# uricchio/2DSFS-scan

Measured on AMD Instinct MI355X. Metric: genomic windows/s (T2D+T1D+Fst) at 20 kb, n1=n2=50; HBM GB/s fraction, higher is better.
Workload: dtype f64

## Files before the change

2dsfs-scan_amd/csrc/sfs2d_kernels.hpp:

```cpp
#pragma once

#include <type_traits>
#include <hip/hip_runtime.h>

#include <cmath>
#include <cstdint>

#include "sfs2d.h"

namespace sfs2dk {

constexpr int WAVE = 64;
constexpr int BLOCK = 256;
constexpr int SBLOCK = 512;
constexpr int BLOCK1 = 512;
constexpr int FBLOCK = 1024;
constexpr int KBLOCK = 512;
constexpr int LNX_N = 1 << 20;
constexpr int LNT = 512;
constexpr int LNF = 256;
__host__ __device__ inline int wl_rtn(int n1p, int n2p) { return 2 * (n1p > n2p ? n1p : n2p) + 2; }
constexpr int RCPN = 512;
#ifndef SFS2D_ABL
#define SFS2D_ABL 0
// ... 500 lines not shown
                                          uint2* __restrict__ slots, uint32_t* __restrict__ bins,
                                          uint32_t* __restrict__ bcount, uint32_t* __restrict__ err_word, int hr,
                                          const double2* __restrict__ rcp_g, unsigned long long* __restrict__ fsum) {
  __shared__ uint32_t sh_b2;
  __shared__ unsigned long long sh_fst[FST ? 2 * FST_R * FST_LDS : 1];
  __shared__ double2 sh_rcp[FST ? RCPN / 2 : 1];
  __shared__ uint32_t sh_wlo;
  static_assert(!JNT || (DO_BG && LDS_HIST && !DO_BINS && !FILT && !FST), "JNT: histogram / segmentation passes only");
  if (JNT) hr = 1;
  STAMP(20);
  BLK_STAMP(0, 0);
  uint32_t* gh = repl + ((size_t)(ti % REPL) * P.nchrom + t.chrom) * (size_t)P.nh;
  const int lane0 = threadIdx.x & (WAVE - 1);
  const int hsh = LDS_HIST ? (hr == 4 ? 2 : 0) : 0;
  const int rep = lane0 & (hr - 1);
  const int trash = P.nh * hr + lane0;
  if (FST) {
    for (int k = threadIdx.x; k < 2 * FST_R * FST_LDS; k += BLOCK1) sh_fst[k] = 0ull;
    for (int k = threadIdx.x; k < RCPN / 2; k += BLOCK1) sh_rcp[k] = rcp_g[k];
    if (threadIdx.x == 0) sh_wlo = DO_SEG ? wid_fast(P, pos[t.begin]) : div_fast(P, t.begin - t.cb);
  }
  if (DO_BG) {
    if (LDS_HIST) {
      const int nz = P.nh * hr + WAVE + (JNT ? P.nb2 : 0);
      uint4* const z4 = reinterpret_cast<uint4*>(sh_hist);
      for (int k = threadIdx.x; k < (nz >> 2); k += BLOCK1) z4[k] = make_uint4(0u, 0u, 0u, 0u);
      if ((int)threadIdx.x < (nz & 3)) sh_hist[(nz & ~3) + (int)threadIdx.x] = 0u;
    }
    if (threadIdx.x == 0) sh_b2 = 0u;
  }
  if (DO_SEG) {
    const uint32_t wf = wid_fast(P, pos[t.begin]);
    const uint32_t lo = t.begin == t.cb ? 0u : wf + 1u;
    const uint32_t hi = t.end == t.ce ? t.nslots : wid_fast(P, pos[t.end]);
    for (uint32_t s = lo + threadIdx.x; s < hi; s += BLOCK1)
      if (s != wf) slots[(size_t)t.sbase + s] = make_uint2(0u, 0u);
  }
  if (DO_BG || FST || DO_SEG) __syncthreads();
  const uint32_t wlo = FST ? sh_wlo : 0u;
  const int frep = threadIdx.x & (FST_R - 1);
  auto fst_add = [&](uint32_t wid, double num, double den) {
    const unsigned long long qn = fst_fixed(num, P.fst_scale), qd = fst_fixed(den, P.fst_scale);
    if ((qn | qd) == 0ull) return;
    const uint32_t j = wid - wlo;
    if (j < (uint32_t)FST_LDS) {
      atomicAdd(&sh_fst[2 * (j * FST_R + frep)], qn);
      atomicAdd(&sh_fst[2 * (j * FST_R + frep) + 1], qd);
    } else {
      atomicAdd(&fsum[2 * ((size_t)t.sbase + wid)], qn);
      atomicAdd(&fsum[2 * ((size_t)t.sbase + wid) + 1], qd);
    }
  };
  const bool pos_filter = FILT && (P.has_start || P.has_end);
  const bool need_pos = DO_SEG || pos_filter;
  const bool filt = FILT && P.ann_want >= 0;
  const int lane = threadIdx.x & (WAVE - 1);
  uint32_t err = 0, b2 = 0;
  STAMP(21);

  KParams Q = P;
  if (!JNT) {
    Q.n1 = vreg(P.n1); Q.n2 = vreg(P.n2); Q.n1p = vreg(P.n1p); Q.n2p = vreg(P.n2p); Q.nb2 = vreg(P.nb2);
    Q.fold_thr = vreg(P.fold_thr); Q.h1a = vreg(P.h1a); Q.h1b = vreg(P.h1b);
    Q.wmag = vreg(P.wmag); Q.wsh1 = vreg(P.wsh1); Q.wsh2 = vreg(P.wsh2);
  }
  auto process = [&](auto EDGE_C, auto FAST_C, uint32_t i0, const uint4& cv, const uint4& pv, const uint2& av,
                     uint32_t wprev, uint32_t wnext) {
    constexpr bool EDGE = decltype(EDGE_C)::value, FAST = decltype(FAST_C)::value;
    const uint32_t cc[4] = {cv.x, cv.y, cv.z, cv.w};
    const uint32_t pp[4] = {pv.x, pv.y, pv.z, pv.w};
    const uint32_t aa[4] = {av.x & 0xffffu, av.x >> 16, av.y & 0xffffu, av.y >> 16};
    uint32_t w[4];
    if (DO_SEG) {
#pragma unroll
      for (int k = 0; k < 4; ++k) w[k] = wid_fast(Q, pp[k]);
    }
    uint32_t bw[4];
    uint32_t segcode = 0;
    uint32_t fw[4];
    bool fm[4];
#pragma unroll
    for (int k = 0; k < 4; ++k) {
      const uint32_t i = i0 + k;
      const bool in = EDGE ? (i >= t.begin) & (i < t.end) : true;
      bool var_ok = in, pos_ok = true;
      if (filt) var_ok = in & ((int)aa[k] == P.ann_want);
      if (pos_filter) {
        const long long p = (long long)pp[k];
        pos_ok = (!P.has_start | (p >= P.start_pos)) & (!P.has_end | (p <= P.end_pos));
      }
      int k2all, u1a, u1b;
      bw[k] = FAST ? classify_fast(Q, cc[k], var_ok, pos_ok, k2all, u1a, u1b)
                   : classify(P, cc[k], var_ok, pos_ok, err, k2all, u1a, u1b);
      if (FST) {
        fw[k] = DO_SEG ? w[k] : div_fast(Q, i - t.cb);
        fm[k] = in & (k2all >= 0) & (DO_SEG | (fw[k] < t.nslots));
      }
      if (DO_BG) {
        if (LDS_HIST) {
          atomicAdd(&sh_hist[(in & (k2all >= 0)) ? (k2all << hsh) + rep : trash], 1u);
          atomicAdd(&sh_hist[(in & (u1a >= 0)) ? ((Q.h1a + u1a) << hsh) + rep : trash], 1u);
          atomicAdd(&sh_hist[(in & (u1b >= 0)) ? ((Q.h1b + u1b) << hsh) + rep : trash], 1u);
        } else if (in) {
          if (k2all >= 0) atomicAdd(&gh[k2all], 1u);
          if (u1a >= 0) atomicAdd(&gh[P.h1a + u1a], 1u);
          if (u1b >= 0) atomicAdd(&gh[P.h1b + u1b], 1u);
        }
        b2 += (in & (bin_k2(bw[k]) != 0)) ? 1u : 0u;
      }
      if (DO_SEG) {
        const uint32_t qp = k ? w[k - 1] : wprev;
        const uint32_t qn = k < 3 ? w[k + 1] : wnext;
        const bool first = in & ((i == t.cb) | (qp != w[k]));
        const bool last = in & ((i + 1 == t.ce) | (qn != w[k]));
        segcode |= (first ? 1u : 0u) << (2 * k) | (last ? 2u : 0u) << (2 * k);
      }
      __builtin_amdgcn_sched_barrier(0);
    }
    if (FST) {
#pragma unroll
      for (int k = 0; k < 4; ++k) {
        double nk, dk;
        fst_snp(cc[k], fm[k], rcp_g, nk, dk);
        if (fm[k]) fst_add(fw[k], nk, dk);
      }
    }
    if (DO_SEG && segcode) {
      for (uint32_t c = segcode; c; c &= c - 1) {
        const int bit = __builtin_ctz(c), k = bit >> 1;
        const uint32_t wk = k == 0 ? w[0] : k == 1 ? w[1] : k == 2 ? w[2] : w[3];
        uint32_t* sl = reinterpret_cast<uint32_t*>(slots + ((size_t)t.sbase + wk));
        sl[bit & 1] = i0 + k + 1u;
      }
    }
    if (DO_BINS) {
      if (!EDGE || (i0 >= t.begin && i0 + 4 <= t.end)) {
        *reinterpret_cast<uint4*>(bins + i0) = make_uint4(bw[0], bw[1], bw[2], bw[3]);
      } else {
#pragma unroll
        for (int k = 0; k < 4; ++k)
          if (i0 + k >= t.begin && i0 + k < t.end) bins[i0 + k] = bw[k];
      }
    }
  };

  constexpr bool FASTOK = !FILT && (!DO_BG || LDS_HIST);
  const uint32_t s2 = (uint32_t)hsh + 2u;
  uint32_t* const hist_l = sh_hist + rep;
  uint32_t* const h1a_l = hist_l + ((uint32_t)P.h1a << hsh);
  uint32_t* const h1b_l = hist_l + ((uint32_t)P.h1b << hsh);
  uint32_t* const trash_p = sh_hist + trash;
  uint32_t* const jh_l = sh_hist + P.nh * hr + WAVE;
  const uint32_t n2p1 = vreg(P.n2 + 1), nb2m1 = vreg(P.nb2 - 1), n1pm1 = vreg(P.n1p - 1), n2pm1 = vreg(P.n2p - 1);
  auto process_fast = [&](uint32_t i0, const uint4& cv, const uint4& pv, uint32_t wprev, uint32_t wnext) {
    const uint32_t cc[4] = {cv.x, cv.y, cv.z, cv.w};
    const uint32_t pp[4] = {pv.x, pv.y, pv.z, pv.w};
    uint32_t w[4], bw[4];
    if (DO_SEG) {
#pragma unroll
      for (int k = 0; k < 4; ++k) w[k] = wid_fast(Q, pp[k]);
    }
    uint32_t fw[4];
    bool fm[4];
#pragma unroll
    for (int k = 0; k < 4; ++k) {
      uint32_t c = cc[k];
      asm volatile("" : "+v"(c));
      const uint32_t r1 = c & 0xffu, a1 = (c >> 8) & 0xffu, r2 = (c >> 16) & 0xffu, a2 = c >> 24;
      const bool sw = (int)(a1 + a2) > Q.fold_thr;
      const uint32_t x1 = sw ? r1 : a1, x2 = sw ? r2 : a2;
      const uint32_t k2 = __umul24(x1, n2p1) + x2;
      const bool in2 = k2 != 0u, last = k2 == nb2m1;
      const uint32_t g1 = min(a1, (uint32_t)Q.n1 - a1), g2 = min(a2, (uint32_t)Q.n2 - a2);
      const uint32_t f1 = g1 - 1u < n1pm1 ? g1 : 0u, f2 = g2 - 1u < n2pm1 ? g2 : 0u;
      bw[k] = (last ? B_LAST : k2) | (f1 << 16) | (f2 << 23) | B_VAR;
      if (DO_BG && !(SFS2D_ABL & 64)) {
        atomicAdd(in2 ? (uint32_t*)((char*)hist_l + (k2 << s2)) : trash_p, 1u);
        atomicAdd(a1 ? (uint32_t*)((char*)h1a_l + (a1 << s2)) : trash_p, 1u);
        atomicAdd(a2 ? (uint32_t*)((char*)h1b_l + (a2 << s2)) : trash_p, 1u);
        b2 += (in2 & !last) ? 1u : 0u;
      }
      if (FST) {
        fw[k] = DO_SEG ? w[k] : div_fast(Q, i0 + k - t.cb);
        fm[k] = in2 & (DO_SEG | (fw[k] < t.nslots));
      }
    }
    if (FST) {
      double sn = 0.0, sd = 0.0;
      uint32_t wc = fw[0];
#pragma unroll
      for (int k = 0; k < 4; ++k) {
        double nk, dk;
        fst_snp(cc[k], fm[k], sh_rcp, nk, dk);
        if (k && fw[k] != wc) {
          fst_add(wc, sn, sd);
          sn = 0.0; sd = 0.0; wc = fw[k];
        }
        sn += nk; sd += dk;
      }
      fst_add(wc, sn, sd);
    }
    if (DO_SEG && wprev != wnext) {
#pragma unroll
      for (int k = 0; k < 4; ++k) {
        const uint32_t qp = k ? w[k - 1] : wprev, qn = k < 3 ? w[k + 1] : wnext;
        uint32_t* sl = reinterpret_cast<uint32_t*>(slots + ((size_t)t.sbase + w[k]));
        if (qp != w[k]) sl[0] = i0 + k + 1u;
        if (qn != w[k]) sl[1] = i0 + k + 1u;
      }
    }
    if (DO_BINS) *reinterpret_cast<uint4*>(bins + i0) = make_uint4(bw[0], bw[1], bw[2], bw[3]);
  };

  constexpr uint32_t LSNP = 4;
  typedef __attribute__((address_space(3))) uint32_t lds_u32;
  const uint32_t kmA = vreg(P.kmul << 8), kmR = P.kmul, fthr = (uint32_t)P.fold_thr;
  const uint32_t jhb = vreg((uint32_t)(uintptr_t)((lds_u32*)jh_l)), h2b = vreg((uint32_t)(uintptr_t)((lds_u32*)sh_hist));
  auto jnt_fast = [&](uint32_t i0, const uint4& cv, const uint4& pv, uint32_t wprev, uint32_t wnext) {
    const uint32_t cc[4] = {cv.x, cv.y, cv.z, cv.w};
    const uint32_t pp[4] = {pv.x, pv.y, pv.z, pv.w};
    if (!(SFS2D_ABL & 64)) {
      uint32_t ka[4], kr[4], sm[4];
#pragma unroll
      for (int k = 0; k < 4; ++k) {
        ka[k] = __builtin_amdgcn_udot4(cc[k], kmA, 0u, false);
        kr[k] = __builtin_amdgcn_udot4(cc[k], kmR, 0u, false);
        sm[k] = __builtin_amdgcn_udot4(cc[k], 0x01000100u, 0u, false);
      }
      asm volatile("" : "+v"(ka[0]), "+v"(ka[1]), "+v"(ka[2]), "+v"(ka[3]), "+v"(kr[0]), "+v"(kr[1]), "+v"(kr[2]),
                        "+v"(kr[3]), "+v"(sm[0]), "+v"(sm[1]), "+v"(sm[2]), "+v"(sm[3]));
#pragma unroll
      for (int k = 0; k < 4; ++k) {
        if (ka[k] != 0u)
          __hip_atomic_fetch_add((lds_u32*)(uintptr_t)(jhb + (ka[k] << 2)), 1u, __ATOMIC_RELAXED, __HIP_MEMORY_SCOPE_WORKGROUP);
        if (((int)sm[k] > (int)fthr) & (kr[k] != 0u))
          __hip_atomic_fetch_add((lds_u32*)(uintptr_t)(h2b + (kr[k] << 2)), 1u, __ATOMIC_RELAXED, __HIP_MEMORY_SCOPE_WORKGROUP);
      }
    }
    if (DO_SEG && wprev != wnext) {
      uint32_t w[LSNP];
#pragma unroll
      for (int k = 0; k < (int)LSNP; ++k) w[k] = wid_fast(P, pp[k]);
#pragma unroll
      for (int k = 0; k < (int)LSNP; ++k) {
        const uint32_t qp = k ? w[k - 1] : wprev, qn = k < (int)LSNP - 1 ? w[k + 1] : wnext;
        uint32_t* sl = reinterpret_cast<uint32_t*>(slots + ((size_t)t.sbase + w[k]));
        if (qp != w[k]) sl[0] = i0 + k + 1u;
        if (qn != w[k]) sl[1] = i0 + k + 1u;
      }
    }
  };

  constexpr uint32_t STEP = LSNP * BLOCK1;
  const uint32_t ab = t.begin & ~3u, alast = (t.end - 1u) & ~3u;
  constexpr bool NEED_C = DO_BG || DO_BINS || FST;
  struct StepIn {
    uint4 c, p;
    uint2 a;
    uint32_t x;
  };
  const uint32_t tbytes = (alast + 4u - ab) * 4u;
  const __amdgpu_buffer_rsrc_t crs = __builtin_amdgcn_make_buffer_rsrc(const_cast<uint32_t*>(counts + ab), (short)0, (int)tbytes, 0x00020000);
  const __amdgpu_buffer_rsrc_t prs = __builtin_amdgcn_make_buffer_rsrc(const_cast<uint32_t*>(pos + ab), (short)0, (int)tbytes, 0x00020000);
  const __amdgpu_buffer_rsrc_t chr_rs =
      __builtin_amdgcn_make_buffer_rsrc(const_cast<uint32_t*>(pos + t.cb), (short)0, (int)((t.ce - t.cb) * 4u), 0x00020000);
  const int lane_off = (int)(LSNP * 4u * threadIdx.x);
  const uint32_t wave_snp = LSNP * WAVE * (uint32_t)__builtin_amdgcn_readfirstlane((int)(threadIdx.x >> 6));
  const uint32_t xlane_off = lane < WAVE / 2 ? 0u - 4u : LSNP * WAVE * 4u;
  auto load_step = [&](uint32_t base) {
    StepIn x;
    const int off = (int)(base - ab) * 4 + lane_off;
    x.c = NEED_C ? __builtin_bit_cast(uint4, __builtin_amdgcn_raw_buffer_load_b128(crs, off, 0, 0)) : make_uint4(0, 0, 0, 0);
    x.p = need_pos ? __builtin_bit_cast(uint4, __builtin_amdgcn_raw_buffer_load_b128(prs, off, 0, 0)) : make_uint4(0, 0, 0, 0);
    x.a = filt ? *reinterpret_cast<const uint2*>(ann + min(base + LSNP * threadIdx.x, alast)) : make_uint2(0, 0);
    x.x = 0;
    if (DO_SEG) {
      const uint32_t wb4 = base < t.end ? (base + wave_snp - t.cb) * 4u : (t.ce - t.cb) * 4u + 4u;
      x.x = __builtin_amdgcn_raw_buffer_load_b32(chr_rs, (int)(wb4 + xlane_off), 0, 0);
    }
    return x;
  };
  auto body = [&](uint32_t base, const StepIn& cur) {
    const uint32_t ia = base + LSNP * threadIdx.x;
    const uint2 aav = cur.a;
    const bool edge = base < t.begin || base + STEP > t.end || base <= t.cb || base + STEP >= t.ce;
    uint32_t wpa = 0, wna = 0;
    if (DO_SEG) {
      uint32_t pprev = dpp_keep<0x138>(cur.x, cur.p.w);
      uint32_t pnext = dpp_keep<0x130>(cur.x, cur.p.x);
      if (edge) {
        const uint32_t none = (t.ce - t.cb) * 4u;
        const uint32_t ni = ia + LSNP;
        const bool edge_next = lane == WAVE - 1 || ni >= t.end;
        const uint32_t op = (lane == 0 && ia > t.cb) ? (min(ia, alast + 4u) - 1u - t.cb) * 4u : none;
        const uint32_t on = (edge_next && ni < t.ce) ? (ni - t.cb) * 4u : none;
        const uint32_t xp = __builtin_amdgcn_raw_buffer_load_b32(chr_rs, (int)op, 0, 0);
        const uint32_t xn = __builtin_amdgcn_raw_buffer_load_b32(chr_rs, (int)on, 0, 0);
        if (lane == 0) pprev = xp;
        if (edge_next) pnext = xn;
      }
      wpa = wid_fast(P, pprev);
      wna = wid_fast(P, pnext);
    }
    auto nc1 = [](uint32_t c) { return __builtin_amdgcn_udot4(c, 0x00000101u, 0u, false); };
    auto nc2 = [](uint32_t c) { return __builtin_amdgcn_udot4(c, 0x01010000u, 0u, false); };
    auto any_bad = [&]() -> bool {
      const uint4 ca = cur.c;
      const uint32_t m1 = max(max(nc1(ca.x), nc1(ca.y)), max(nc1(ca.z), nc1(ca.w)));
      const uint32_t m2 = max(max(nc2(ca.x), nc2(ca.y)), max(nc2(ca.z), nc2(ca.w)));
      return __ballot((m1 > (uint32_t)P.n1) | (m2 > (uint32_t)P.n2)) != 0ull;
    };
    using T_ = std::true_type;
    using F_ = std::false_type;
    bool exact = !FASTOK || edge;
    int nc_ok = P.nc_ok;
    asm volatile("" : "+s"(nc_ok));
    if (!exact && !nc_ok) exact = any_bad();
    if (exact) process(T_{}, F_{}, ia, cur.c, cur.p, aav, wpa, wna);
    else {
#ifdef SFS2D_MARK
      asm volatile("; HOT_BEGIN");
#endif
      if (SFS2D_ABL & 128)
        asm volatile("" ::"v"(cur.c.x), "v"(cur.c.y), "v"(cur.c.z), "v"(cur.c.w), "v"(cur.p.x), "v"(cur.p.w), "v"(wpa), "v"(wna));
      else if constexpr (JNT) jnt_fast(ia, cur.c, cur.p, wpa, wna);
      else process_fast(ia, cur.c, cur.p, wpa, wna);
#ifdef SFS2D_MARK
      asm volatile("; HOT_END");
#endif
    }
  };
#if SFS2D_PREP_PREFETCH >= 2
  StepIn bufA = load_step(ab), bufB = load_step(ab + STEP);
  for (uint32_t base = ab; base < t.end; base += 2 * STEP) {
    body(base, bufA);
    bufA = load_step(base + 2 * STEP);
    if (base + STEP >= t.end) break;
    body(base + STEP, bufB);
    bufB = load_step(base + 3 * STEP);
  }
#else
  StepIn nxt = load_step(ab);
  for (uint32_t base = ab; base < t.end; base += STEP) {
#if SFS2D_PREP_PREFETCH
    const StepIn cur = nxt;
    if (base + STEP < t.end) nxt = load_step(base + STEP);
#else
    const StepIn cur = base == ab ? nxt : load_step(base);
#endif
    body(base, cur);
  }
#endif
  STAMP(22);
  if (err) atomicOr(err_word, err);
  if (DO_BG && !JNT) {
    b2 = wave_sum_u(b2);
    if (lane == 0 && b2) atomicAdd(&sh_b2, b2);
  }
  if (DO_BG || FST) __syncthreads();
  if (JNT) {
    const uint32_t n2p1 = (uint32_t)P.n2 + 1u;
    uint32_t bs = 0;
    for (int k = threadIdx.x; k < P.nb2; k += BLOCK1) {
      const uint32_t j = jh_l[k];
      const uint32_t x1 = __umulhi((uint32_t)k, P.n2inv), x2 = (uint32_t)k - x1 * n2p1;
      if (j) {
        if (x1) atomicAdd(&sh_hist[P.h1a + (int)x1], j);
        if (x2) atomicAdd(&sh_hist[P.h1b + (int)x2], j);
      }
      const uint32_t v = sh_hist[k] + ((int)(x1 + x2) <= P.fold_thr ? j : 0u);
      if (k) sh_hist[k] = v;
      if (k >= 1 && k <= P.nb2 - 2) bs += v;
    }
    bs = wave_sum_u(bs);
    if (lane == 0 && bs) atomicAdd(&sh_b2, bs);
    __syncthreads();
  }
  if (FST)
    for (int j = threadIdx.x; j < FST_LDS; j += BLOCK1) {
      unsigned long long qn = 0, qd = 0;
#pragma unroll
      for (int r = 0; r < FST_R; ++r) {
        qn += sh_fst[2 * (j * FST_R + r)];
        qd += sh_fst[2 * (j * FST_R + r) + 1];
      }
      if (qn | qd) {
        atomicAdd(&fsum[2 * ((size_t)t.sbase + wlo + j)], qn);
        atomicAdd(&fsum[2 * ((size_t)t.sbase + wlo + j) + 1], qd);
      }
    }
  if (DO_BG) {
    if (LDS_HIST)
      for (int k = threadIdx.x; k < P.nh; k += BLOCK1) {
        uint32_t v;
        if (hr == 4) {
// ... 1089 lines not shown
  __builtin_amdgcn_s_barrier();
#endif
  BLK_STAMP(1, 1);
}

template <int CTRL>
__device__ __forceinline__ double mdpp_d(double v) {
  const unsigned long long u = __double_as_longlong(v);
  const int lo = __builtin_amdgcn_mov_dpp((int)(u & 0xffffffffull), CTRL, 0xf, 0xf, false);
  const int hi = __builtin_amdgcn_mov_dpp((int)(u >> 32), CTRL, 0xf, 0xf, false);
  return __longlong_as_double((long long)(((unsigned long long)(uint32_t)hi << 32) | (uint32_t)lo));
}
__device__ __forceinline__ void wave_sum2_halves(double a, double b, double& s2, double& sa, double& sb) {
  a += mdpp_d<0xB1>(a);  b += mdpp_d<0xB1>(b);
  a += mdpp_d<0x4E>(a);  b += mdpp_d<0x4E>(b);
  a += mdpp_d<0x141>(a); b += mdpp_d<0x141>(b);
  a += mdpp_d<0x140>(a); b += mdpp_d<0x140>(b);
  s2 = (readlane_d(a, 0) + readlane_d(a, 16)) + (readlane_d(a, 32) + readlane_d(a, 48));
  sa = readlane_d(b, 0) + readlane_d(b, 16);
  sb = readlane_d(b, 32) + readlane_d(b, 48);
}
__device__ __forceinline__ double wave_sum1(double v) {
  v += mdpp_d<0xB1>(v);
  v += mdpp_d<0x4E>(v);
  v += mdpp_d<0x141>(v);
  v += mdpp_d<0x140>(v);
  return (readlane_d(v, 0) + readlane_d(v, 16)) + (readlane_d(v, 32) + readlane_d(v, 48));
}

__device__ __forceinline__ double swap16_d(double v, bool upper) {
  const unsigned long long u = __double_as_longlong(v);
  const auto lo = __builtin_amdgcn_permlane16_swap((uint32_t)(u & 0xffffffffull), (uint32_t)(u & 0xffffffffull), false, false);
  const auto hi = __builtin_amdgcn_permlane16_swap((uint32_t)(u >> 32), (uint32_t)(u >> 32), false, false);
  const uint32_t l = upper ? lo[1] : lo[0], h = upper ? hi[1] : hi[0];
  return __longlong_as_double((long long)(((unsigned long long)h << 32) | l));
}
__device__ __forceinline__ double swap32_d(double v, bool upper) {
  const unsigned long long u = __double_as_longlong(v);
  const auto lo = __builtin_amdgcn_permlane32_swap((uint32_t)(u & 0xffffffffull), (uint32_t)(u & 0xffffffffull), false, false);
  const auto hi = __builtin_amdgcn_permlane32_swap((uint32_t)(u >> 32), (uint32_t)(u >> 32), false, false);
  const uint32_t l = upper ? lo[1] : lo[0], h = upper ? hi[1] : hi[0];
  return __longlong_as_double((long long)(((unsigned long long)h << 32) | l));
}
__device__ __forceinline__ double row_sum_d(double v) {
  v += mdpp_d<0xB1>(v);
  v += mdpp_d<0x4E>(v);
  v += mdpp_d<0x141>(v);
  v += mdpp_d<0x140>(v);
  return v;
}
__device__ __forceinline__ double wave_sum_all(double v) {
  v = row_sum_d(v);
  v = swap16_d(v, false) + swap16_d(v, true);
  return swap32_d(v, false) + swap32_d(v, true);
}
__device__ __forceinline__ void wave_sum_halves_all(double v, double& a, double& b) {
  v = row_sum_d(v);
  v = swap16_d(v, false) + swap16_d(v, true);
  a = swap32_d(v, false);
  b = swap32_d(v, true);
}

__device__ __forceinline__ void swap32_pair(double x, double y, double& xo, double& yo) {
  const unsigned long long u = __double_as_longlong(x), v = __double_as_longlong(y);
  const auto lo = __builtin_amdgcn_permlane32_swap((uint32_t)u, (uint32_t)v, false, false);
  const auto hi = __builtin_amdgcn_permlane32_swap((uint32_t)(u >> 32), (uint32_t)(v >> 32), false, false);
  xo = __longlong_as_double((long long)(((unsigned long long)hi[0] << 32) | lo[0]));
  yo = __longlong_as_double((long long)(((unsigned long long)hi[1] << 32) | lo[1]));
}
__device__ __forceinline__ void swap16_pair(double x, double y, double& xo, double& yo) {
  const unsigned long long u = __double_as_longlong(x), v = __double_as_longlong(y);
  const auto lo = __builtin_amdgcn_permlane16_swap((uint32_t)u, (uint32_t)v, false, false);
  const auto hi = __builtin_amdgcn_permlane16_swap((uint32_t)(u >> 32), (uint32_t)(v >> 32), false, false);
  xo = __longlong_as_double((long long)(((unsigned long long)hi[0] << 32) | lo[0]));
  yo = __longlong_as_double((long long)(((unsigned long long)hi[1] << 32) | lo[1]));
}
__device__ __forceinline__ double wave_sum5(double a, double h, double f1, double f2, uint32_t lane) {
  double x, y;
  swap32_pair(a, f2, x, y);
  const double r1 = x + y;
  swap32_pair(f1, h, x, y);
  const double r2 = lane < 32 ? x + y : y;
  const double r3 = x;
  swap16_pair(r1, r2, x, y);
  const double q = x + y;
  swap16_pair(r3, r3, x, y);
  const double t = x + y;
  const bool odd = lane & 1u;
  double z = odd ? t : q;
  z += mdpp_d<0xB1>(odd ? q : t);
  z += mdpp_d<0x4E>(z);
  z += mdpp_d<0x124>(z);
  z += mdpp_d<0x128>(z);
  return z;
}

__device__ __forceinline__ void wave_sum3(double a, double b, double c, double& sa, double& sb, double& sc) {
  double x, y;
  swap32_pair(a, b, x, y);
  const double r1 = x + y;
  swap32_pair(c, c, x, y);
  const double r2 = x + y;
  swap16_pair(r1, r2, x, y);
  double q = x + y;
  q += mdpp_d<0xB1>(q);
  q += mdpp_d<0x4E>(q);
  q += mdpp_d<0x124>(q);
  q += mdpp_d<0x128>(q);
  sa = readlane_d(q, 0);
  sc = readlane_d(q, 16);
  sb = readlane_d(q, 32);
}

extern "C" __device__ int sfs2d_llvm_writelane(int v, int l, int old) __asm("llvm.amdgcn.writelane.i32");
__device__ __forceinline__ uint32_t wlane(uint32_t v, int l, uint32_t old) {
  return (uint32_t)sfs2d_llvm_writelane((int)__builtin_amdgcn_readfirstlane((int)v), l, (int)old);
}


__device__ __forceinline__ void lds_copy_d(double* dst, const double* __restrict__ src, int n) {
  constexpr int U = 8;
  for (int k0 = threadIdx.x; k0 < n; k0 += U * SBLOCK) {
    double v[U];
#pragma unroll
    for (int j = 0; j < U; ++j) v[j] = k0 + j * SBLOCK < n ? src[k0 + j * SBLOCK] : 0.0;
#pragma unroll
    for (int j = 0; j < U; ++j)
      if (k0 + j * SBLOCK < n) dst[k0 + j * SBLOCK] = v[j];
  }
}

template <bool P16, bool FUSED, int FST, bool CNT, bool GATE = false>
__device__ __forceinline__ void scan_w_small(double* ldsd, uint32_t wgi, uint32_t nwg, SCAN_W_ARGS) {
  constexpr bool FSTIN = FST >= 2;
  constexpr bool FMASK = FST == 3;
  static_assert(!FSTIN || CNT, "Fst in the scan reads the counts");
  static_assert(!GATE || CNT, "the gate is a property of the counts the scan classifies");
  constexpr int DT = LNT;
  constexpr int R1U = R1;
  constexpr int NWV = SBLOCK / WAVE;
  constexpr int SB = 8;
  __shared__ BgHead sh_hb;
  __shared__ double sh_bd[NWV][3][SB];
  __shared__ uint32_t sh_bu[NWV][5][SB];
  __shared__ unsigned long long sh_bf[NWV][FST ? 2 : 1][SB];
  STAMP(10);
  BLK_STAMP(1, 0);
  const int tid = threadIdx.x;
  const int wv = __builtin_amdgcn_readfirstlane(tid >> 6);
  const int lane = tid & (WAVE - 1);
  const Chunk ch = chunks[wgi];
  const int bg = bg_per_chrom ? (int)ch.chrom : 0;

  double* LPl = ldsd;
  double* Dt = LPl + ((P.nt + 1) & ~1);
  double* Ft = Dt + DT;
  double2* RT = reinterpret_cast<double2*>(Ft + LNF);
  const int rtn = FSTIN ? P.rtn : 0;
  uint32_t* HB = reinterpret_cast<uint32_t*>(RT + rtn);
  const int h2w = P16 ? ((P.nb2 + 1) / 2 + 3) & ~3 : (P.nb2 + 3) & ~3;
  const int h1w = R1 * (P.n1p + 1), h1wb = R1 * (P.n2p + 1);
  const int per = (h2w + h1w + h1wb + 3) & ~3;
  uint32_t* W = HB + wv * per;
  uint32_t* H1a = W + h2w;
  uint32_t* H1b = H1a + h1w;
  const uint32_t rep = lane & (R1U - 1);

  auto bounds = [&](uint32_t s, uint2 sr, Win& w, bool live) {
    if (mode_bp) {
      w.has = live && sr.x != 0u;
      w.b = sr.x - 1u;
      w.e = sr.y;
    } else {
      w.has = live;
      w.b = ch.cb + (ch.wid_lo + (s - ch.slot_lo)) * P.ws;
      w.e = w.b + P.ws;
    }
    const __amdgpu_buffer_rsrc_t rr = window_rows(bins, w.has ? w.b : 0u, w.has ? w.e : 0u, P.nm1);
    uint32_t lo = (uint32_t)lane * 4u;
    asm volatile("" : "+v"(lo));
#pragma unroll
    for (int j = 0; j < 8; ++j) w.u[j] = __builtin_amdgcn_raw_buffer_load_b32(rr, (int)lo + 256 * j, 0, 0);
  };
  uint32_t s = ch.slot_lo + ch.first + wv;
  const bool active = s < ch.slot_hi;
  const uint2 sr0 = (active && mode_bp) ? slots[s] : make_uint2(0, 0);
  const uint32_t npool = ch.pool & 0xffffu, pool = ch.pool >> 16;
  const bool dyn = ch.slot_lo + ch.nstatic < ch.slot_hi;
  const uint32_t dbase = ch.slot_lo + ch.nstatic + pool;
  uint32_t* myctr = ctr + (((size_t)cpar * P.nchrom + ch.chrom) * CTR_POOLS + pool) * CTR_STRIDE;
  uint32_t gq1 = 0, gq = 0;
  if (active && dyn && lane == 0) {
    gq1 = atomicAdd(myctr, 1u);
    gq = atomicAdd(myctr, 1u);
  }
  if (wgi == 0)
    for (int k = tid; k < P.nchrom * CTR_POOLS; k += SBLOCK) ctr[((size_t)(1 - cpar) * P.nchrom * CTR_POOLS + k) * CTR_STRIDE] = 0u;

  static_assert(LNT == SBLOCK && LNF <= SBLOCK, "one D and at most one F double per thread");
  const double dfv0 = dfg[tid], dfv1 = tid < LNF ? dfg[LNT + tid] : 0.0;
  const double2 rtv = (FSTIN && tid < rtn) ? reinterpret_cast<const double2*>(dfg + 2 * LNT)[tid] : make_double2(0.0, 0.0);
  auto stage_fst = [&]() {
    if (FSTIN && tid < rtn) RT[tid] = rtv;
  };
  BgHead hb;
  const size_t rs = (size_t)P.nchrom * P.nh;
  const uint32_t* Rc = repl + (size_t)par * REPL * rs + (size_t)ch.chrom * P.nh;
  if (!FUSED) {
    double lsv = 0.0;
    int4 my_node = make_int4(0, 0, -1, 0);
    uint32_t bc = 0u;
    Bg1D o{};
    if (sliced) {
      if (tid < nleaves) lsv = leafsum[(size_t)bg * nleaves + tid];
      if (tid < nnodes) my_node = nodes[tid];
      if (tid == 0) { bc = bcount[(size_t)par * P.nchrom + bg]; o = bg1d[bg]; }
    }
    lds_copy_d(LPl, LPg + (size_t)bg * P.nt, P.nt);
    if (tid < DT) Dt[tid] = dfv0;
    if (tid < LNF) Ft[tid] = dfv1;
    stage_fst();
    if (sliced) {
      const bool writer = ch.first == 0 && (int)ch.chrom == write_chrom;
      double* lsum = reinterpret_cast<double*>(HB);
      if (tid < nleaves) lsum[tid] = lsv;
      __syncthreads();
      for (int l = 0; l < nlevels; ++l) {
        if (my_node.z == l) lsum[nleaves + tid] = lsum[my_node.x] + lsum[my_node.y];
        __syncthreads();
      }
      if (tid == 0) {
        const double B2 = (double)bc;
        uint32_t flags = o.flags;
        if (B2 == 0.0) flags |= BGF_B2_ZERO;
        const int M2 = P.nb2 - 2;
        if (M2 >= 1 && B2 != 0.0) {
          const double S = (nleaves + nnodes) ? lsum[nleaves + nnodes - 1] : 0.0;
          const double padj = 1.0 - S;
          if (padj < -1e-15) {
            flags |= BGF_NAN2;
          } else if (fabs(padj) > 1e-15) {
            const double l2 = log(padj);
            LPl[M2] = l2;
            if (writer) { tab[(size_t)bg * P.nt + M2].lp = l2; LPg[(size_t)bg * P.nt + M2] = l2; }
          }
        }
        BgHead h;
        h.B2 = B2; h.B1a = o.B1a; h.B1b = o.B1b; h.flags = flags; h.pad = 0;
        sh_hb = h;
        if (writer) head[bg] = h;
      }
      if (wgi == 0)
        for (int c = tid; c < P.nchrom; c += SBLOCK) bcount[(size_t)(1 - par) * P.nchrom + c] = 0u;
      __syncthreads();
      hb = sh_hb;
    } else {
      hb = head[bg];
    }
  } else {
    if (tid < DT) Dt[tid] = dfv0;
    if (tid < LNF) Ft[tid] = dfv1;
    stage_fst();
    fused_table(P.nb2, P.nh, P.nt, P.n1p, P.n2p, P.n1, P.n2, P.t1a, P.t1b, P.nchrom, ch.chrom,
                ch.first == 0 && (int)ch.chrom == write_chrom, bg,
                Rc, rs, repl, bcount, par, tab, LPg, head, LPl, HB, leaves, nleaves, nodes, nnodes, nlevels, lnx,
                &sh_hb, reinterpret_cast<double*>(HB) + 1536, HB + FUSED_VCNT);
    hb = sh_hb;
  }
  for (int k = lane; k < per / 4; k += WAVE) reinterpret_cast<uint4*>(W)[k] = make_uint4(0, 0, 0, 0);
  if (tid == 0) LPl[0] = 0.0;
  __syncthreads();
  if (FUSED) {
    uint32_t* Ro = repl + (size_t)(1 - par) * REPL * rs;
    const size_t tot = (size_t)REPL * rs, share = (tot + nwg - 1) / nwg;
    const size_t lo = (size_t)wgi * share, hi = lo + share < tot ? lo + share : tot;
    for (size_t k = lo + tid; k < hi; k += SBLOCK) Ro[k] = 0u;
    if (wgi == 0)
      for (int c = tid; c < P.nchrom; c += SBLOCK) bcount[(size_t)(1 - par) * P.nchrom + c] = 0u;
  }
  if (!active) return;
  const bool filt = P.ann_want >= 0;
  const bool half1d = P.n1p <= 31 && P.n2p <= 31;
  const uint32_t zflags = bg_zero_flags(hb);
  const bool nan2 = hb.flags & BGF_NAN2, nan1a = hb.flags & BGF_NAN1A, nan1b = hb.flags & BGF_NAN1B;
  uint32_t* const H1a_l = H1a + rep;
  uint32_t* const H1b_l = H1b + rep;
  const uint32_t one1 = P16 ? 0x10000u : 1u;
  typedef __attribute__((address_space(3))) uint32_t lds_u32;
  uint32_t a1b = (uint32_t)(uintptr_t)((lds_u32*)H1a_l), a2b = (uint32_t)(uintptr_t)((lds_u32*)H1b_l);
  asm volatile("" : "+v"(a1b), "+v"(a2b));
  uint32_t awb = (uint32_t)(uintptr_t)((lds_u32*)W);
  asm volatile("" : "+s"(awb));
  typedef double d2v __attribute__((ext_vector_type(2)));
  typedef __attribute__((address_space(3))) d2v lds_d2;
  const uint32_t rtb = (uint32_t)(uintptr_t)((lds_d2*)RT);
  uint32_t jb = 0;
  double fl2 = 0.0, fla = 0.0, flb = 0.0;
  auto flush = [&]() {
    MARK(30);
    if (SFS2D_ABL & 512) { jb = 0; return; }
    uint32_t ln = __builtin_amdgcn_mbcnt_hi(~0u, __builtin_amdgcn_mbcnt_lo(~0u, 0u));
    asm volatile("" : "+v"(ln));
    const bool mine = ln < jb;
    const int jl = ln & (SB - 1);
    const double B2 = sh_bd[wv][0][jl], Ba = sh_bd[wv][1][jl], Bb = sh_bd[wv][2][jl];
    const uint32_t Bs = sh_bu[wv][0][jl], Bsb = sh_bu[wv][1][jl], Bn2 = sh_bu[wv][2][jl], Bn1 = sh_bu[wv][3][jl],
                   Bnv = sh_bu[wv][4][jl];
    const uint32_t nsnp = Bnv & 0xffffu;
    const bool empty = nsnp == 0u;
    const uint32_t wid = ch.wid_lo + (Bs - ch.slot_lo);
    const uint32_t Bse = Bsb + nsnp;
    WinOut w;
    w.snp_count = Bnv >> 16; w.n2 = Bn2 & 0xffffu; w.n2_all = Bn2 >> 16; w.n1a = Bn1 & 0xffffu; w.n1b = Bn1 >> 16;
    w.t2d = 2.0 * (B2 - __dmul_rn((double)w.n2, fl2));
    w.t1a = 2.0 * (Ba - __dmul_rn((double)w.n1a, fla));
    w.t1b = 2.0 * (Bb - __dmul_rn((double)w.n1b, flb));
    const bool exact = mine && !empty &&
                       (nsnp == 0xffffu || suspect_zero(w.t2d, w.n2) ||
                        suspect_zero(w.t1a, w.n1a) || suspect_zero(w.t1b, w.n1b));
    if (nan2) w.t2d = __builtin_nan("");
    if (nan1a) w.t1a = __builtin_nan("");
    if (nan1b) w.t1b = __builtin_nan("");
    if (empty) { w.t2d = 0.0; w.t1a = 0.0; w.t1b = 0.0; }
    if (mine && !exact)
      if (!(SFS2D_ABL & 8)) write_rec(out + Bs, ch.chrom, wid, empty ? 0u : Bsb, empty ? 0u : Bse, w, empty ? SFS2D_W_EMPTY : zflags);
    if (mine) {
      if (FSTIN) {
        const double fx = __longlong_as_double((long long)sh_bf[wv][0][jl]);
        const double fy = __longlong_as_double((long long)sh_bf[wv][FST ? 1 : 0][jl]);
        fst_out[Bs] = fy >= 0x1p-10 ? fx / fy : __builtin_nan("");
      } else if (FST) {
        const long long fx = (long long)sh_bf[wv][0][jl], fy = (long long)sh_bf[wv][FST ? 1 : 0][jl];
        fst_out[Bs] = fy != 0 ? (double)fx / (double)fy : __builtin_nan("");
        reinterpret_cast<ulonglong2*>(fsum)[Bs] = make_ulonglong2(0ull, 0ull);
      }
    }
      if (mine && mode_bp && !FSTIN && !exact) {
        uint32_t z = 0u;
        asm volatile("" : "+v"(z));
        slots[Bs] = make_uint2(z, z);
      }
    MARK(31);
    for (unsigned long long m = __ballot(exact); m; m &= m - 1) {
      const int l = __builtin_ctzll(m);
      const uint32_t xs = __builtin_amdgcn_readlane(Bs, l), xb = __builtin_amdgcn_readlane(Bsb, l);
      const uint32_t xn = __builtin_amdgcn_readlane(Bnv, l) & 0xffffu;
      const uint32_t xe = xn != 0xffffu ? xb + xn : (mode_bp ? slots[xs].y : xb + P.ws);
      WinOut x;
      if (FUSED) {
        x = eval_exact<WAVE, P16, R1, CNT>(P, bins, xb, xe,
                                      TabFused{LPl, Rc, rs, P.nb2, P.n1, P.n2, P.n1p, P.h1a, P.h1b, P.t1a, P.t1b}, hb,
                                      lnx, W, H1a, H1b, nullptr, nullptr);
      } else {
        x = eval_exact<WAVE, P16, R1, CNT>(P, bins, xb, xe, TabLocal{tab + (size_t)bg * P.nt, LPl}, hb, lnx, W, H1a, H1b,
                                      nullptr, nullptr);
      }
      if (lane == 0) {
        write_rec(out + xs, ch.chrom, ch.wid_lo + (xs - ch.slot_lo), xb, xe, x, zflags);
        atomicAdd(err_word + 1, 1u);
      }
      group_sync<WAVE>();
    }
    jb = 0;
  };
  auto put_u = [&](uint32_t slot, uint32_t b, uint32_t nsnp, uint32_t n2, uint32_t n1a, uint32_t n1b, uint32_t nvar,
                   uint32_t nlast) {
    sh_bu[wv][0][jb] = slot;
    sh_bu[wv][1][jb] = b;
    sh_bu[wv][2][jb] = min(n2, 0xffffu) | (min(n2 + nlast, 0xffffu) << 16);
    sh_bu[wv][3][jb] = min(n1a, 0xffffu) | (min(n1b, 0xffffu) << 16);
    sh_bu[wv][4][jb] = min(nsnp, 0xffffu) | (min(nvar, 0xffffu) << 16);
  };
  auto put = [&](uint32_t slot, uint32_t b, uint32_t nsnp, uint32_t n2, uint32_t n1a, uint32_t n1b, uint32_t nvar,
                 uint32_t nlast, double s2, double sa, double sb, ulonglong2 fq) {
    if (lane == 0) {
      sh_bd[wv][0][jb] = s2; sh_bd[wv][1][jb] = sa; sh_bd[wv][2][jb] = sb;
      if (FST) { sh_bf[wv][0][jb] = fq.x; sh_bf[wv][FST ? 1 : 0][jb] = fq.y; }
      put_u(slot, b, nsnp, n2, n1a, n1b, nvar, nlast);
    }
  };
  typedef __attribute__((address_space(3))) double lds_f64;
  constexpr unsigned long long OWN5 = 1ull | (1ull << 33) | (1ull << 48) | (FSTIN ? (1ull << 16) | (1ull << 32) : 0ull);
  uint32_t sdst;
  {
    double* d = lane == 0 ? &sh_bd[wv][0][0] : lane == 33 ? &sh_bd[wv][1][0] : lane == 48 ? &sh_bd[wv][2][0]
              : lane == 16 ? reinterpret_cast<double*>(&sh_bf[wv][0][0])
                           : reinterpret_cast<double*>(&sh_bf[wv][FST ? 1 : 0][0]);
    sdst = (uint32_t)(uintptr_t)((lds_f64*)d);
  }
  asm volatile("" : "+v"(sdst));
  auto put5 = [&](double v, ulonglong2 fq) {
    if ((OWN5 >> lane) & 1ull) ((lds_f64*)(uintptr_t)(sdst + 8u * jb))[0] = v;
    if (FST == 1 && lane == 0) { sh_bf[wv][0][jb] = fq.x; sh_bf[wv][FST ? 1 : 0][jb] = fq.y; }
  };


  auto pool_slot = [&](uint32_t g) -> uint32_t {
    const uint32_t j = __builtin_amdgcn_readfirstlane(g);
    return dyn && dbase + npool * j < ch.slot_hi ? dbase + npool * j : ch.slot_hi;
  };
  Win cur;
  bounds(s, sr0, cur, true);
  uint32_t s1 = pool_slot(gq1);
  uint2 sr1 = (mode_bp && s1 < ch.slot_hi) ? slots[s1] : make_uint2(0, 0);
  uint2 srs = make_uint2(0, 0);
  STAMP(11);
  int it = 0;
  for (;;) {
  while (s < ch.slot_hi) {
    const bool fill = jb + 1u < (uint32_t)SB;
    const bool more = s1 < ch.slot_hi;
    const uint2 sr1u = make_uint2(__builtin_amdgcn_readfirstlane(sr1.x), __builtin_amdgcn_readfirstlane(sr1.y));
    Win nxt;
    nxt.has = false;
    bounds(s1, sr1u, nxt, more && fill);
    const uint32_t s2 = more ? pool_slot(gq) : ch.slot_hi;
    const uint2 sr2 = (mode_bp && s2 < ch.slot_hi) ? slots[s2] : make_uint2(0, 0);
    if (s2 < ch.slot_hi && lane == 0) gq = atomicAdd(myctr, 1u);
    if (!cur.has) {
      put(s, 0u, 0u, 0u, 0u, 0u, 0u, 0u, 0.0, 0.0, 0.0, make_ulonglong2(0ull, 0ull));
      ++jb;
      cur = nxt;
      s = s1; srs = sr1u;
      s1 = s2; sr1 = sr2;
      if (!fill) break;
      continue;
    }
    const uint32_t nsnp = cur.e - cur.b;
    const int lim = (int)nsnp - lane;
    const bool clampd = nsnp > (uint32_t)(LNT - 1);
    double acc2 = 0.0;
    double fA = 0.0, fP = 0.0, fM = 0.0;
    uint32_t n2 = 0, n1a = 0, n1b = 0, nlast = 0, nvar = 0;
    uint32_t kw[8];
    auto fst_load = [&](uint32_t w0, uint32_t w1, double2 (&fq)[4]) {
      if (FSTIN) {
        const uint32_t ww[2] = {w0, w1};
#pragma unroll
        for (int q = 0; q < 2; ++q) {
          const uint32_t w = ww[q];
          const uint32_t n1c = __builtin_amdgcn_udot4(w, 0x00000101u, 0u, false);
          const uint32_t n2c = __builtin_amdgcn_udot4(w, 0x01010000u, 0u, false);
          uint32_t a1 = __builtin_amdgcn_ubfe(w, 8, 8), a2 = w >> 24;
          if (FMASK) {
            const bool ok = min(n1c, n2c) >= 2u;
            a1 = ok ? a1 : 0u;
            a2 = ok ? a2 : 0u;
          }
          d2v r1, r2;
          if (SFS2D_ABL & 16) {
            r1.x = (double)n1c; r1.y = (double)n1c; r2.x = (double)n2c; r2.y = (double)n2c;
          } else {
            r1 = *(const lds_d2*)(uintptr_t)(rtb + 16u * n1c);
            r2 = *(const lds_d2*)(uintptr_t)(rtb + 16u * n2c);
          }
          const double d1 = (double)a1, d2 = (double)a2;
          fq[2 * q] = make_double2(d1 * r1.x, fma(d1, d1, -d1) * r1.y);
          fq[2 * q + 1] = make_double2(d2 * r2.x, fma(d2, d2, -d2) * r2.y);
        }
      }
    };
    auto pair = [&](uint32_t w0, uint32_t w1, int j, bool keep, const double2 (&fq)[4]) {
      const uint32_t ww[2] = {w0, w1};
      uint32_t rk[2], kk[2], ov[2], xs[2];
      bool in2[2];
#pragma unroll
      for (int q = 0; q < 2; ++q) {
        const uint32_t w = ww[q];
        uint32_t k2, gp;
        if (CNT) cls_k2g<GATE>(P, w, k2, gp);
        else { k2 = bin_k2(w); gp = bin_g1(w) | (bin_g2(w) << 16); }
        in2[q] = k2 != 0u;
        n2 += __popcll(__ballot(in2[q]));
        const uint32_t x = (CNT ? k2 : w) << 4;
        const uint32_t word = P16 ? (k2 >> 1) : k2;
        uint32_t one2 = 1u;
        if (P16) asm("v_lshlrev_b32 %0, %1, 1" : "=v"(one2) : "v"(x));
        const uint32_t wa = awb + word * 4u;
        uint32_t o = one2;
        if (in2[q] && !(SFS2D_ABL & 1))
          o = __hip_atomic_fetch_add((lds_u32*)(uintptr_t)wa, one2, __ATOMIC_RELAXED, __HIP_MEMORY_SCOPE_WORKGROUP);
        ov[q] = o;
        xs[q] = x;
        kk[q] = k2;
        if (keep) kw[(j + q) & 7] = word;
        constexpr int BS1 = 4 * R1;
        static_assert(BS1 <= 64, "the multiplier must be an inline constant");
        uint32_t u1, u2;
        asm("v_mad_u32_u16 %0, %1, %3, %2" : "=v"(u1) : "v"(gp), "v"(a1b), "n"(BS1));
        asm("v_mad_u32_u16 %0, %1, %3, %2 op_sel:[1,0,0,0]" : "=v"(u2) : "v"(gp), "v"(a2b), "n"(BS1));
        if (!(SFS2D_ABL & 2)) {
          __hip_atomic_fetch_add((lds_u32*)(uintptr_t)u1, one1, __ATOMIC_RELAXED, __HIP_MEMORY_SCOPE_WORKGROUP);
          __hip_atomic_fetch_add((lds_u32*)(uintptr_t)u2, one1, __ATOMIC_RELAXED, __HIP_MEMORY_SCOPE_WORKGROUP);
        }
      }
      if (FSTIN) {
        const double a0 = fq[0].y + fq[1].y, a1 = fq[2].y + fq[3].y;
        const double p0 = fq[0].x + fq[1].x, p1 = fq[2].x + fq[3].x;
        if (j == 0) {
          fA = a0 + a1;
          fP = p0 + p1;
          fM = fma(fq[2].x, fq[3].x, fq[0].x * fq[1].x);
        } else {
          fA += a0 + a1;
          fP += p0 + p1;
          fM = fma(fq[2].x, fq[3].x, fma(fq[0].x, fq[1].x, fM));
        }
      }
#pragma unroll
      for (int q = 0; q < 2; ++q)
        rk[q] = in2[q] ? (P16 ? __builtin_amdgcn_ubfe(ov[q], xs[q], 16) : ov[q]) : 0u;
      double d[2], lp[2];
#pragma unroll
      for (int q = 0; q < 2; ++q) {
        static_assert(8 * WAVE <= LNT, "a rank of the first 8 rows must stay inside the D table");
        d[q] = (SFS2D_ABL & 4) ? (double)rk[q] : Dt[keep ? rk[q] : min(rk[q], (uint32_t)LNT - 1u)];
        lp[q] = (SFS2D_ABL & 4) ? (double)kk[q] : LPl[kk[q]];
      }
      const double t = (d[0] - lp[0]) + (d[1] - lp[1]);
      acc2 = j == 0 ? t : acc2 + t;
    };
    MARK(19);
#pragma unroll
    for (int j = 0; j < 8; j += 2)
      if (64 * j < (int)nsnp) {
        const uint32_t w0 = (CNT || 64 * j < lim) ? cur.u[j] : 0u, w1 = (CNT || 64 * (j + 1) < lim) ? cur.u[j + 1] : 0u;
        double2 fq[4];
        fst_load(w0, w1, fq);
        pair(w0, w1, j, true, fq);
      }
    MARK(20);
    if (nsnp > 8 * WAVE) {
      const uint32_t* qb = bins + cur.b;
      uint32_t ln = (uint32_t)lane;
      asm volatile("" : "+v"(ln));
      if (CNT) {
        const __amdgpu_buffer_rsrc_t rr = window_rows(bins, cur.b, cur.e, P.nm1);
        int vo = (int)(ln * 4u) + 256 * 8;
        uint32_t x0 = __builtin_amdgcn_raw_buffer_load_b32(rr, vo, 0, 0), x1 = __builtin_amdgcn_raw_buffer_load_b32(rr, vo + 256, 0, 0);
        for (int j = 8; 64 * j < (int)nsnp; j += 2) {
          const uint32_t w0 = x0, w1 = x1;
          double2 fq[4];
          fst_load(w0, w1, fq);
          vo += 512;
          x0 = __builtin_amdgcn_raw_buffer_load_b32(rr, vo, 0, 0);
          x1 = __builtin_amdgcn_raw_buffer_load_b32(rr, vo + 256, 0, 0);
          pair(w0, w1, j, false, fq);
        }
        asm volatile("" ::"v"(x0), "v"(x1));
      } else {
        uint32_t x0 = 64 * 8 < lim ? qb[ln + 64 * 8] : 0u, x1 = 64 * 9 < lim ? qb[ln + 64 * 9] : 0u;
        for (int j = 8; 64 * j < (int)nsnp; j += 2) {
          const uint32_t w0 = 64 * j < lim ? x0 : 0u, w1 = 64 * (j + 1) < lim ? x1 : 0u;
          x0 = 64 * (j + 2) < lim ? qb[ln + 64u * (j + 2)] : 0u;
          x1 = 64 * (j + 3) < lim ? qb[ln + 64u * (j + 3)] : 0u;
          double2 fq[4];
          pair(w0, w1, j, false, fq);
        }
      }
    }
    MARK(22);
    if (GATE ? (!P.fold || filt) : (!P.fold || !CNT || !P.nc_ok)) {
      for (uint32_t i0 = cur.b; i0 < cur.e; i0 += WAVE) {
        const uint32_t w = i0 + lane < cur.e ? snp_word<CNT>(P, bins, i0 + lane) : 0u;
        nlast += __popcll(__ballot((w & B_LAST) != 0u));
        nvar += __popcll(__ballot((w & B_VAR) != 0u));
      }
    }
    if (!filt) nvar = nsnp;
    ulonglong2 fq = make_ulonglong2(0ull, 0ull);
    if (FST == 1 && lane == 0) fq = reinterpret_cast<const ulonglong2*>(fsum)[s];
    if (it == 0) STAMP(12);
    MARK(23);
    group_sync<WAVE>();
    if (clampd) {
      constexpr uint32_t L1 = LNT - 1;
      const double fl = (double)L1 * lnx[L1];
      for (int k = lane; k < h2w; k += WAVE) {
        const uint32_t v = W[k];
        const uint32_t xa = P16 ? (v & 0xffffu) : v, xb = P16 ? (v >> 16) : 0u;
        if (xa > L1) acc2 += (double)xa * lnx_of(lnx, xa) - fl;
        if (xb > L1) acc2 += (double)xb * lnx_of(lnx, xb) - fl;
      }
    }
    if (nsnp <= 8 * WAVE) {
#pragma unroll
      for (int j = 0; j < 8; ++j)
        if (64 * j < (int)nsnp) W[kw[j]] = 0u;
    } else {
      uint4* q = reinterpret_cast<uint4*>(W);
      for (int k = lane; k < h2w / 4; k += WAVE) q[k] = make_uint4(0, 0, 0, 0);
    }
    MARK(24);
    double acca = 0.0, accb = 0.0;
    constexpr uint32_t S1 = P16 ? 16u : 0u;
    const uint32_t slots = 128u * ((nsnp + 127u) / 128u);
    auto take1 = [&](uint32_t* H, int k) -> uint32_t {
      if (SFS2D_ABL & 32) return (uint32_t)k;
      return take_replicas<R1U>(H + k * R1, S1);
    };
    if (half1d) {
      const bool pa = lane < 32;
      const int k = lane & 31, np = pa ? P.n1p : P.n2p;
      uint32_t x = 0;
      if (k <= np) {
        x = take1(pa ? H1a : H1b, k);
        if (k >= 1 && k < np && x) acca = xlnx<LNF>(x, Ft, lnx) - (double)x * LPl[(pa ? P.t1a : P.t1b) + k];
      }
      n1a = slots - (uint32_t)__builtin_amdgcn_readlane((int)x, 0) - (uint32_t)__builtin_amdgcn_readlane((int)x, P.n1p);
      n1b = slots - (uint32_t)__builtin_amdgcn_readlane((int)x, 32) -
            (uint32_t)__builtin_amdgcn_readlane((int)x, 32 + P.n2p);
    } else {
      uint32_t xa[2] = {0u, 0u}, xb[2] = {0u, 0u};
#pragma unroll
      for (int j = 0; j < 2; ++j) {
        const int k = lane + WAVE * j;
        if (k <= P.n1p) {
          const uint32_t x = take1(H1a, k);
          xa[j] = x;
          if (k >= 1 && k < P.n1p && x) acca += xlnx<LNF>(x, Ft, lnx) - (double)x * LPl[P.t1a + k];
        }
        if (k <= P.n2p) {
          const uint32_t x = take1(H1b, k);
          xb[j] = x;
          if (k >= 1 && k < P.n2p && x) accb += xlnx<LNF>(x, Ft, lnx) - (double)x * LPl[P.t1b + k];
        }
      }
      const uint32_t ea = P.n1p >= WAVE ? (uint32_t)__builtin_amdgcn_readlane((int)xa[1], P.n1p - WAVE)
                                        : (uint32_t)__builtin_amdgcn_readlane((int)xa[0], P.n1p);
      const uint32_t eb = P.n2p >= WAVE ? (uint32_t)__builtin_amdgcn_readlane((int)xb[1], P.n2p - WAVE)
                                        : (uint32_t)__builtin_amdgcn_readlane((int)xb[0], P.n2p);
      n1a = slots - (uint32_t)__builtin_amdgcn_readlane((int)xa[0], 0) - ea;
      n1b = slots - (uint32_t)__builtin_amdgcn_readlane((int)xb[0], 0) - eb;
    }
    if (it == 0) STAMP(13);
    MARK(25);
    if (half1d) {
      const double m2 = 2.0 * fM;
      const double v = (SFS2D_ABL & 256) ? acc2 + acca + (FSTIN ? fA - m2 + fP : 0.0)
                                         : wave_sum5(acc2, acca, FSTIN ? fA - m2 : 0.0, FSTIN ? fP - m2 : 0.0, (uint32_t)lane);
      MARK(26);
      put5(v, fq);
      if (lane == 0) put_u(s, cur.b, nsnp, n2, n1a, n1b, nvar, nlast);
      if ((uint32_t)lane == jb) {
        fl2 = lnx[min(n2, 0xffffu)];
        fla = lnx[min(n1a, 0xffffu)];
        flb = lnx[min(n1b, 0xffffu)];
      }
    } else {
      const double s2 = wave_sum_all(acc2);
      const double sa = wave_sum_all(acca), sb = wave_sum_all(accb);
      if (FSTIN) {
        const double m2 = 2.0 * fM;
        fq = make_ulonglong2((unsigned long long)__double_as_longlong(wave_sum_all(fA - m2)),
                             (unsigned long long)__double_as_longlong(wave_sum_all(fP - m2)));
      }
      MARK(26);
      put(s, cur.b, nsnp, n2, n1a, n1b, nvar, nlast, s2, sa, sb, fq);
      if ((uint32_t)lane == jb) {
        fl2 = lnx[min(n2, 0xffffu)];
        fla = lnx[min(n1a, 0xffffu)];
        flb = lnx[min(n1b, 0xffffu)];
      }
    }
    ++jb;
    group_sync<WAVE>();
    if (it == 0) STAMP(14);
    MARK(28);
    ++it;
// ... 299 lines not shown
```

Measured before the change: 901.6 million.

## Fold reciprocal address into udot4 and shortcut window-id lookup at edges

Reorders the LDS layout so the D table sits at the base and the reciprocal table lies at a fixed offset from it. A single udot4 then computes the per-population sample count scaled by 16 plus the base address, and the fixed distance goes into the ds_read immediate, which removes separate count and address arithmetic in the Fst path. Window ids at segment edges are derived from a threshold compare when the whole wave spans at most one window boundary, avoiding wid_fast, and the non-Fst path no longer computes ids for every SNP. The classification calls are also hoisted before the atomic loop to improve scheduling. The layout swap relies on the LDS sizing staying equal and on the immediate-offset bound.

```diff
diff --git a/2dsfs-scan_amd/csrc/sfs2d_kernels.hpp b/2dsfs-scan_amd/csrc/sfs2d_kernels.hpp
--- a/2dsfs-scan_amd/csrc/sfs2d_kernels.hpp
+++ b/2dsfs-scan_amd/csrc/sfs2d_kernels.hpp
@@ -676,11 +676,21 @@
   uint32_t* const trash_p = sh_hist + trash;
   uint32_t* const jh_l = sh_hist + P.nh * hr + WAVE;
   const uint32_t n2p1 = vreg(P.n2 + 1), nb2m1 = vreg(P.nb2 - 1), n1pm1 = vreg(P.n1p - 1), n2pm1 = vreg(P.n2p - 1);
+  auto edge_wids = [&](const KParams& K, const uint32_t (&pp)[4], uint32_t wprev, uint32_t wnext, uint32_t (&w)[4]) {
+    if (__ballot(wnext - wprev > 1u) == 0ull) {
+      const uint32_t thr = (wprev + 1u) * P.ws;
+#pragma unroll
+      for (int k = 0; k < 4; ++k) w[k] = wprev + (pp[k] > thr ? 1u : 0u);
+    } else {
+#pragma unroll
+      for (int k = 0; k < 4; ++k) w[k] = wid_fast(K, pp[k]);
+    }
+  };
   auto process_fast = [&](uint32_t i0, const uint4& cv, const uint4& pv, uint32_t wprev, uint32_t wnext) {
     const uint32_t cc[4] = {cv.x, cv.y, cv.z, cv.w};
     const uint32_t pp[4] = {pv.x, pv.y, pv.z, pv.w};
     uint32_t w[4], bw[4];
-    if (DO_SEG) {
+    if (DO_SEG && FST) {
 #pragma unroll
       for (int k = 0; k < 4; ++k) w[k] = wid_fast(Q, pp[k]);
     }
@@ -725,6 +735,7 @@
       fst_add(wc, sn, sd);
     }
     if (DO_SEG && wprev != wnext) {
+      if (!FST) edge_wids(Q, pp, wprev, wnext, w);
 #pragma unroll
       for (int k = 0; k < 4; ++k) {
         const uint32_t qp = k ? w[k - 1] : wprev, qn = k < 3 ? w[k + 1] : wnext;
@@ -763,8 +774,7 @@
     }
     if (DO_SEG && wprev != wnext) {
       uint32_t w[LSNP];
-#pragma unroll
-      for (int k = 0; k < (int)LSNP; ++k) w[k] = wid_fast(P, pp[k]);
+      edge_wids(P, pp, wprev, wnext, w);
 #pragma unroll
       for (int k = 0; k < (int)LSNP; ++k) {
         const uint32_t qp = k ? w[k - 1] : wprev, qn = k < (int)LSNP - 1 ? w[k + 1] : wnext;
@@ -2160,12 +2170,14 @@
   const Chunk ch = chunks[wgi];
   const int bg = bg_per_chrom ? (int)ch.chrom : 0;
 
-  double* LPl = ldsd;
-  double* Dt = LPl + ((P.nt + 1) & ~1);
+  constexpr bool DOTA = FSTIN && !FMASK;
+  const int rtn = FSTIN ? P.rtn : 0;
+  const int lpn = (P.nt + 1) & ~1;
+  double* Dt = DOTA ? ldsd : ldsd + lpn;
   double* Ft = Dt + DT;
   double2* RT = reinterpret_cast<double2*>(Ft + LNF);
-  const int rtn = FSTIN ? P.rtn : 0;
-  uint32_t* HB = reinterpret_cast<uint32_t*>(RT + rtn);
+  double* LPl = DOTA ? reinterpret_cast<double*>(RT + rtn) : ldsd;
+  uint32_t* HB = DOTA ? reinterpret_cast<uint32_t*>(LPl + lpn) : reinterpret_cast<uint32_t*>(RT + rtn);
   const int h2w = P16 ? ((P.nb2 + 1) / 2 + 3) & ~3 : (P.nb2 + 3) & ~3;
   const int h1w = R1 * (P.n1p + 1), h1wb = R1 * (P.n2p + 1);
   const int per = (h2w + h1w + h1wb + 3) & ~3;
@@ -2302,6 +2314,10 @@
   typedef double d2v __attribute__((ext_vector_type(2)));
   typedef __attribute__((address_space(3))) d2v lds_d2;
   const uint32_t rtb = (uint32_t)(uintptr_t)((lds_d2*)RT);
+  typedef __attribute__((address_space(3))) double lds_dbl;
+  constexpr uint32_t RT_OFF = (uint32_t)((DT + LNF) * sizeof(double));
+  static_assert(RT_OFF < 65536u, "the reciprocals' distance from D must fit a ds_read's immediate offset");
+  const uint32_t dtv = (uint32_t)(uintptr_t)((lds_dbl*)Dt);
   uint32_t jb = 0;
   double fl2 = 0.0, fla = 0.0, flb = 0.0;
   auto flush = [&]() {
@@ -2447,20 +2463,25 @@
 #pragma unroll
         for (int q = 0; q < 2; ++q) {
           const uint32_t w = ww[q];
-          const uint32_t n1c = __builtin_amdgcn_udot4(w, 0x00000101u, 0u, false);
-          const uint32_t n2c = __builtin_amdgcn_udot4(w, 0x01010000u, 0u, false);
           uint32_t a1 = __builtin_amdgcn_ubfe(w, 8, 8), a2 = w >> 24;
-          if (FMASK) {
-            const bool ok = min(n1c, n2c) >= 2u;
-            a1 = ok ? a1 : 0u;
-            a2 = ok ? a2 : 0u;
-          }
           d2v r1, r2;
-          if (SFS2D_ABL & 16) {
-            r1.x = (double)n1c; r1.y = (double)n1c; r2.x = (double)n2c; r2.y = (double)n2c;
+          if (!DOTA || (SFS2D_ABL & 16)) {
+            const uint32_t n1c = __builtin_amdgcn_udot4(w, 0x00000101u, 0u, false);
+            const uint32_t n2c = __builtin_amdgcn_udot4(w, 0x01010000u, 0u, false);
+            if (FMASK) {
+              const bool ok = min(n1c, n2c) >= 2u;
+              a1 = ok ? a1 : 0u;
+              a2 = ok ? a2 : 0u;
+            }
+            if (SFS2D_ABL & 16) {
+              r1.x = (double)n1c; r1.y = (double)n1c; r2.x = (double)n2c; r2.y = (double)n2c;
+            } else {
+              r1 = *(const lds_d2*)(uintptr_t)(rtb + 16u * n1c);
+              r2 = *(const lds_d2*)(uintptr_t)(rtb + 16u * n2c);
+            }
           } else {
-            r1 = *(const lds_d2*)(uintptr_t)(rtb + 16u * n1c);
-            r2 = *(const lds_d2*)(uintptr_t)(rtb + 16u * n2c);
+            r1 = *(const lds_d2*)(uintptr_t)(__builtin_amdgcn_udot4(w, 0x00001010u, dtv, false) + RT_OFF);
+            r2 = *(const lds_d2*)(uintptr_t)(__builtin_amdgcn_udot4(w, 0x10100000u, dtv, false) + RT_OFF);
           }
           const double d1 = (double)a1, d2 = (double)a2;
           fq[2 * q] = make_double2(d1 * r1.x, fma(d1, d1, -d1) * r1.y);
@@ -2472,12 +2493,17 @@
       const uint32_t ww[2] = {w0, w1};
       uint32_t rk[2], kk[2], ov[2], xs[2];
       bool in2[2];
+      uint32_t k2q[2], gpq[2];
+#pragma unroll
+      for (int q = 0; q < 2; ++q) {
+        if (CNT) cls_k2g<GATE>(P, ww[q], k2q[q], gpq[q]);
+        else { k2q[q] = bin_k2(ww[q]); gpq[q] = bin_g1(ww[q]) | (bin_g2(ww[q]) << 16); }
+      }
+      if (CNT) asm volatile("" : "+v"(k2q[0]), "+v"(k2q[1]));
 #pragma unroll
       for (int q = 0; q < 2; ++q) {
         const uint32_t w = ww[q];
-        uint32_t k2, gp;
-        if (CNT) cls_k2g<GATE>(P, w, k2, gp);
-        else { k2 = bin_k2(w); gp = bin_g1(w) | (bin_g2(w) << 16); }
+        const uint32_t k2 = k2q[q], gp = gpq[q];
         in2[q] = k2 != 0u;
         n2 += __popcll(__ballot(in2[q]));
         const uint32_t x = (CNT ? k2 : w) << 4;
@@ -2522,7 +2548,8 @@
 #pragma unroll
       for (int q = 0; q < 2; ++q) {
         static_assert(8 * WAVE <= LNT, "a rank of the first 8 rows must stay inside the D table");
-        d[q] = (SFS2D_ABL & 4) ? (double)rk[q] : Dt[keep ? rk[q] : min(rk[q], (uint32_t)LNT - 1u)];
+        const uint32_t rc = keep ? rk[q] : min(rk[q], (uint32_t)LNT - 1u);
+        d[q] = (SFS2D_ABL & 4) ? (double)rk[q] : Dt[rc];
         lp[q] = (SFS2D_ABL & 4) ? (double)kk[q] : LPl[kk[q]];
       }
       const double t = (d[0] - lp[0]) + (d[1] - lp[1]);
```

Result: faster. 913.0 million (median of 6 runs) (+1.3%).
